# DJjjjhao/FIRA-ICSE

Hardware: NVIDIA B200
Metric: train_commits_per_sec (higher is better)
Workload: dtype bf16

## Files before the change

### fira_icse_b200/csrc/gemm_tc.cu

```cuda
#include <cuda.h>
#include <cudaTypedefs.h>
#include <atomic>
#include <stdlib.h>
#include "common.cuh"
#include "fira_b200.h"

namespace {

constexpr int BM = 128;
constexpr int BK = 64;
constexpr int UMMA_K = 16;
constexpr int NUM_THREADS = 192;

struct TcParams {
  void* C; long ldc; int c_is_bf16;
  int M, N, K;
  const float* bias; const float* rs; const float* rc;
  int relu; int accumulate;
  int splits; int kblocks_per_split;
  int a_kmajor, b_kmajor;
  int rotate;
  int tma_store;
  const __nv_bfloat16* relu_mask;
  float* colsum;
  unsigned long long* probe;
};

std::atomic<unsigned long long*> g_probe{nullptr};

__device__ __forceinline__ void stamp(const TcParams& p, int slot) {
  if (p.probe && blockIdx.x == 0 && blockIdx.y == 0 && blockIdx.z == 0) {
    unsigned long long t;
    asm volatile("mov.u64 %0, %globaltimer;" : "=l"(t));
    p.probe[slot] = t;
  }
}

__device__ __forceinline__ uint32_t smem_addr(const void* p) { return (uint32_t)__cvta_generic_to_shared(p); }

__device__ __forceinline__ void mbar_init(uint32_t bar, uint32_t count) {
  asm volatile("mbarrier.init.shared::cta.b64 [%0], %1;" ::"r"(bar), "r"(count));
}
__device__ __forceinline__ void mbar_expect_tx(uint32_t bar, uint32_t bytes) {
  asm volatile("mbarrier.arrive.expect_tx.shared::cta.b64 _, [%0], %1;" ::"r"(bar), "r"(bytes) : "memory");
}
__device__ __forceinline__ void mbar_wait(uint32_t bar, uint32_t parity) {
  uint32_t ok = 0, spins = 0;
  while (true) {
// ... 9 lines not shown
}
__device__ __forceinline__ void tc_fence_before() { asm volatile("tcgen05.fence::before_thread_sync;" ::: "memory"); }
__device__ __forceinline__ void tc_fence_after() { asm volatile("tcgen05.fence::after_thread_sync;" ::: "memory"); }
__device__ __forceinline__ void umma_commit(uint32_t bar) {
  asm volatile("tcgen05.commit.cta_group::1.mbarrier::arrive::one.shared::cluster.b64 [%0];" ::"r"(bar) : "memory");
}
__device__ __forceinline__ void umma_bf16(uint32_t tmem_d, uint64_t desc_a, uint64_t desc_b, uint32_t idesc,
                                          uint32_t accumulate) {
  asm volatile("{\n\t.reg .pred p;\n\tsetp.ne.b32 p, %4, 0;\n\t"
               "tcgen05.mma.cta_group::1.kind::f16 [%0], %1, %2, %3, p;\n\t}"
               ::"r"(tmem_d), "l"(desc_a), "l"(desc_b), "r"(idesc), "r"(accumulate) : "memory");
}

__device__ __forceinline__ uint64_t make_desc(uint32_t saddr, uint32_t lbo_bytes, uint32_t sbo_bytes) {
  uint64_t d = 0;
  d |= (uint64_t)((saddr >> 4) & 0x3FFF);
  d |= (uint64_t)((lbo_bytes >> 4) & 0x3FFF) << 16;
  d |= (uint64_t)((sbo_bytes >> 4) & 0x3FFF) << 32;
  d |= (uint64_t)1 << 46;
  d |= (uint64_t)2 << 61;
  return d;
}

template <int BN, int STAGES>
__global__ void __launch_bounds__(NUM_THREADS, 2)
gemm_tc_kernel(const __grid_constant__ CUtensorMap tmA, const __grid_constant__ CUtensorMap tmB,
               const __grid_constant__ CUtensorMap tmC, TcParams p) {
  extern __shared__ unsigned char smem_dyn[];
  __shared__ __align__(16) float s_bias[BN], s_rc[BN];
  constexpr uint32_t A_BYTES = BM * BK * 2, B_BYTES = BN * BK * 2, STAGE_BYTES = A_BYTES + B_BYTES;
  __shared__ __align__(8) unsigned long long full_bar[STAGES], empty_bar[STAGES], tmem_full_bar;
  __shared__ uint32_t tmem_base_slot;

  const uint32_t base = (smem_addr(smem_dyn) + 1023u) & ~1023u;
  const int warp = threadIdx.x >> 5, lane = threadIdx.x & 31;
  const int m0 = blockIdx.y * BM, n0 = blockIdx.x * BN;
  const int kb_total = (p.K + BK - 1) / BK;
  const int kb_begin = blockIdx.z * p.kblocks_per_split;
  const int kb_end = min(kb_total, kb_begin + p.kblocks_per_split);
  const int nkb = kb_end - kb_begin;
  if (threadIdx.x == 0) stamp(p, 0);

  const bool do_cs = p.colsum != nullptr && blockIdx.x == 0;
  if (threadIdx.x == 0) {
    for (int s = 0; s < STAGES; ++s) { mbar_init(smem_addr(&full_bar[s]), 1); mbar_init(smem_addr(&empty_bar[s]), do_cs ? 5 : 1); }
    mbar_init(smem_addr(&tmem_full_bar), 1);
    asm volatile("fence.mbarrier_init.release.cluster;" ::: "memory");
    asm volatile("prefetch.tensormap [%0];" ::"l"(&tmA) : "memory");
    asm volatile("prefetch.tensormap [%0];" ::"l"(&tmB) : "memory");
    if (p.tma_store) asm volatile("prefetch.tensormap [%0];" ::"l"(&tmC) : "memory");
  }
  if (warp == 1) {
    asm volatile("tcgen05.alloc.cta_group::1.sync.aligned.shared::cta.b32 [%0], %1;" ::"r"(smem_addr(&tmem_base_slot)), "r"(BN));
    asm volatile("tcgen05.relinquish_alloc_permit.cta_group::1.sync.aligned;");
  }
  tc_fence_before();
  __syncthreads();
  tc_fence_after();
  const uint32_t tmem_acc = tmem_base_slot;
  if (threadIdx.x == 0) stamp(p, 1);
  pdl_wait(); pdl_trigger();
  if (threadIdx.x == 0) stamp(p, 2);

  if (warp == 0 && lane == 0) {
    for (int i = 0; i < nkb; ++i) {
      const int s = i % STAGES;
      const uint32_t ph = (i / STAGES) & 1;
      mbar_wait(smem_addr(&empty_bar[s]), ph ^ 1);
      const uint32_t sa = base + s * STAGE_BYTES, sb = sa + A_BYTES;
      const uint32_t fb = smem_addr(&full_bar[s]);
      mbar_expect_tx(fb, STAGE_BYTES);
      const int kb = p.rotate ? kb_begin + (i + (int)(blockIdx.x + blockIdx.y)) % nkb : kb_begin + i;
      const int k0 = kb * BK;
      if (p.a_kmajor) {
        tma_load_2d(sa, &tmA, k0, m0, fb);
      } else {
        tma_load_2d(sa, &tmA, m0, k0, fb);
        tma_load_2d(sa + 8192, &tmA, m0 + 64, k0, fb);
      }
      if (p.b_kmajor) {
        tma_load_2d(sb, &tmB, k0, n0, fb);
      } else {
#pragma unroll
        for (int j = 0; j < BN / 64; ++j) tma_load_2d(sb + j * 8192, &tmB, n0 + j * 64, k0, fb);
      }
    }
    stamp(p, 3);
  } else if (warp == 1 && lane == 0) {
    const uint32_t idesc = (1u << 4) | (1u << 7) | (1u << 10) | ((p.a_kmajor ? 0u : 1u) << 15) |
                           ((p.b_kmajor ? 0u : 1u) << 16) | ((uint32_t)(BN >> 3) << 17) | ((uint32_t)(BM >> 4) << 24);
    for (int i = 0; i < nkb; ++i) {
      const int s = i % STAGES;
      const uint32_t ph = (i / STAGES) & 1;
      mbar_wait(smem_addr(&full_bar[s]), ph);
      tc_fence_after();
      if (i == 0) stamp(p, 4);
      const uint32_t sa = base + s * STAGE_BYTES, sb = sa + A_BYTES;
#pragma unroll
      for (int k = 0; k < BK / UMMA_K; ++k) {
        const uint64_t da = p.a_kmajor ? make_desc(sa + k * 32, 16, 1024) : make_desc(sa + k * 2048, 8192, 1024);
        const uint64_t db = p.b_kmajor ? make_desc(sb + k * 32, 16, 1024) : make_desc(sb + k * 2048, 8192, 1024);
        umma_bf16(tmem_acc, da, db, idesc, (i > 0 || k > 0) ? 1u : 0u);
      }
      umma_commit(smem_addr(&empty_bar[s]));
    }
    umma_commit(smem_addr(&tmem_full_bar));
    stamp(p, 5);
  } else if (warp >= 2) {
    const int quarter = warp & 3;
    constexpr int HB = BN < 128 ? BN : 128;
    constexpr int PITCH = HB + 4;
    constexpr int LPR = HB / 8;
    constexpr int RPI = 32 / LPR;
    float* stg = reinterpret_cast<float*>(smem_dyn + (base - smem_addr(smem_dyn))) + (size_t)quarter * 32 * PITCH;
    if (do_cs) {
      const int t = quarter * 32 + lane;
      const unsigned char* a_base = smem_dyn + (base - smem_addr(smem_dyn)) + (t >> 6) * 8192 + (t & 7) * 2;
      const int chunk = (t & 63) >> 3;
      float cs = 0.f;
      for (int i = 0; i < nkb; ++i) {
        const int s = i % STAGES;
        mbar_wait(smem_addr(&full_bar[s]), (i / STAGES) & 1);
        const unsigned char* a = a_base + (size_t)s * STAGE_BYTES;
#pragma unroll 8
        for (int k = 0; k < BK; ++k)
          cs += __bfloat162float(*reinterpret_cast<const __nv_bfloat16*>(a + (k >> 3) * 1024 + (k & 7) * 128 + ((chunk ^ (k & 7)) << 4)));
        __syncwarp();
        if (lane == 0) asm volatile("mbarrier.arrive.shared::cta.b64 _, [%0];" ::"r"(smem_addr(&empty_bar[s])) : "memory");
      }
      if (m0 + t < p.M) atomicAdd(p.colsum + m0 + t, cs);
      asm volatile("bar.sync 1, 128;" ::: "memory");
// ... 242 lines not shown
    if (cudaGetDriverEntryPoint("cuTensorMapEncodeTiled", &f, cudaEnableDefault, &q) != cudaSuccess) f = nullptr;
    return (PFN_cuTensorMapEncodeTiled)f;
  }();
  return fn;
}

int make_map(CUtensorMap* map, const void* ptr, long rows, long cols, long ld, int box_cols, int box_rows) {
  PFN_cuTensorMapEncodeTiled enc = get_encode();
  if (!enc) { fira_set_error(FIRA_ERR_CUDA, "gemm_tc: cuTensorMapEncodeTiled unavailable"); return FIRA_ERR_CUDA; }
  cuuint64_t dims[2] = {(cuuint64_t)cols, (cuuint64_t)rows};
  cuuint64_t strides[1] = {(cuuint64_t)ld * 2};
  cuuint32_t box[2] = {(cuuint32_t)box_cols, (cuuint32_t)box_rows};
  cuuint32_t estr[2] = {1, 1};
  CUresult r = enc(map, CU_TENSOR_MAP_DATA_TYPE_BFLOAT16, 2, const_cast<void*>(ptr), dims, strides, box, estr,
                   CU_TENSOR_MAP_INTERLEAVE_NONE, CU_TENSOR_MAP_SWIZZLE_128B, CU_TENSOR_MAP_L2_PROMOTION_L2_128B,
                   CU_TENSOR_MAP_FLOAT_OOB_FILL_NONE);
  if (r != CUDA_SUCCESS) {
    fira_set_error(FIRA_ERR_CUDA, "gemm_tc: cuTensorMapEncodeTiled failed (%d) rows=%ld cols=%ld ld=%ld", (int)r, rows, cols, ld);
    return FIRA_ERR_CUDA;
  }
  return FIRA_OK;
}

template <int BN, int STAGES>
int launch_cfg(const CUtensorMap& ta, const CUtensorMap& tb, const CUtensorMap& tc, const TcParams& p, cudaStream_t st) {
  const size_t smem = (size_t)STAGES * (BM * BK * 2 + BN * BK * 2) + 1024;
  cudaError_t e = cudaFuncSetAttribute(gemm_tc_kernel<BN, STAGES>, cudaFuncAttributeMaxDynamicSharedMemorySize, (int)smem);
  if (e != cudaSuccess) { fira_set_error(FIRA_ERR_CUDA, "gemm_tc attr: %s", cudaGetErrorString(e)); return FIRA_ERR_CUDA; }
  dim3 grid((p.N + BN - 1) / BN, (p.M + BM - 1) / BM, p.splits);
  launch_k(gemm_tc_kernel<BN, STAGES>, dim3(grid), dim3(NUM_THREADS), smem, st, ta, tb, tc, p);
  return FIRA_OK;
}

template <int BN>
int launch(const CUtensorMap& ta, const CUtensorMap& tb, const CUtensorMap& tc, const TcParams& p, cudaStream_t st) {
  const long ctas = (long)((p.N + BN - 1) / BN) * ((p.M + BM - 1) / BM) * p.splits;
  if (ctas > 148) return launch_cfg<BN, (BN == 256 ? 2 : 3)>(ta, tb, tc, p, st);
  return launch_cfg<BN, 4>(ta, tb, tc, p, st);
}

}

extern "C" int fira_debug_set_probe(void* probe) {
  g_probe.store((unsigned long long*)probe, std::memory_order_relaxed);
  return FIRA_OK;
}

namespace {
int gemm_tc_impl(const void* A, long lda, int a_kmajor, const void* B, long ldb, int b_kmajor, void* C, long ldc,
                 int c_is_bf16, int M, int N, int K, const float* bias, const float* rs, const float* rc, int relu,
                 int accumulate, int splits, float* colsum, void* stream, const void* relu_mask = nullptr) {
  FIRA_CHECK_ARG(A && B && C, FIRA_ERR_ARG, "gemm_bf16_tc: null operand");
  FIRA_CHECK_ARG(M > 0 && N > 0 && K > 0, FIRA_ERR_SHAPE, "gemm_bf16_tc: M=%d N=%d K=%d", M, N, K);
  FIRA_CHECK_ARG((lda % 8) == 0 && (ldb % 8) == 0, FIRA_ERR_ALIGN, "gemm_bf16_tc: lda/ldb must be multiples of 8");
  FIRA_CHECK_ARG(fira_aligned16(A) && fira_aligned16(B) && fira_aligned16(C), FIRA_ERR_ALIGN, "gemm_bf16_tc: 16-B alignment");
  FIRA_CHECK_ARG((rs == nullptr) == (rc == nullptr), FIRA_ERR_ARG, "gemm_bf16_tc: rs/rc must come together");
  FIRA_CHECK_ARG(!(splits > 1 && (c_is_bf16 || relu)), FIRA_ERR_ARG, "gemm_bf16_tc: split-K needs fp32 C and no relu");
  cudaStream_t st = (cudaStream_t)stream;
  int BN = N > 128 ? 256 : (N > 64 ? 128 : 64);
  {
    const long mt = (M + BM - 1) / BM;
    const int sp = splits < 1 ? 1 : splits;
    for (int cand = 64; cand < BN; cand *= 2)
      if (mt * ((N + cand - 1) / cand) * sp <= 148) { BN = cand; break; }
  }
  CUtensorMap ta, tb;
  int rc_;
  if (a_kmajor) rc_ = make_map(&ta, A, M, K, lda, BK, BM); else rc_ = make_map(&ta, A, K, M, lda, 64, BK);
  if (rc_) return rc_;
  if (b_kmajor) rc_ = make_map(&tb, B, N, K, ldb, BK, BN); else rc_ = make_map(&tb, B, K, N, ldb, 64, BK);
  if (rc_) return rc_;
  const int kb_total = (K + BK - 1) / BK;
  if (splits < 1) splits = 1;
  if (splits > kb_total) splits = kb_total;
  int per = (kb_total + splits - 1) / splits;
  splits = (kb_total + per - 1) / per;
  const int tma_store = (c_is_bf16 && !accumulate && splits == 1 && (ldc % 8) == 0 && tma_store_on()) ? 1 : 0;
  CUtensorMap tc = ta;
  if (tma_store) {
    rc_ = make_map(&tc, C, M, N, ldc, 64, 32);
    if (rc_) return rc_;
  }
  FIRA_CHECK_ARG(relu_mask == nullptr || tma_store, FIRA_ERR_ARG,
                 "gemm_bf16_tc: the relu mask needs the TMA-store epilogue (bf16 C, no accumulate, no split-K)");
  TcParams p{C, ldc, c_is_bf16, M, N, K, bias, rs, rc, relu, accumulate, splits, per, a_kmajor, b_kmajor, rotate_on() ? 1 : 0,
             tma_store, (const __nv_bfloat16*)relu_mask, colsum,
             g_probe.load(std::memory_order_relaxed)};
  if (splits > 1 && !accumulate) {
    cudaError_t e = cudaMemset2DAsync(C, (size_t)ldc * 4, 0, (size_t)N * 4, (size_t)M, st);
    if (e != cudaSuccess) { fira_set_error(FIRA_ERR_CUDA, "gemm_bf16_tc memset: %s", cudaGetErrorString(e)); return FIRA_ERR_CUDA; }
  }
  if (BN == 256) rc_ = launch<256>(ta, tb, tc, p, st);
  else if (BN == 128) rc_ = launch<128>(ta, tb, tc, p, st);
  else rc_ = launch<64>(ta, tb, tc, p, st);
  if (rc_) return rc_;
  FIRA_CHECK_LAUNCH("fira_gemm_bf16_tc");
  return FIRA_OK;
}
}

extern "C" int fira_gemm_bf16_tc(const void* A, long lda, int a_kmajor, const void* B, long ldb, int b_kmajor, void* C,
                                 long ldc, int c_is_bf16, int M, int N, int K, const float* bias, const float* rs,
                                 const float* rc, int relu, int accumulate, int splits, void* stream) {
  return gemm_tc_impl(A, lda, a_kmajor, B, ldb, b_kmajor, C, ldc, c_is_bf16, M, N, K, bias, rs, rc, relu, accumulate, splits,
                      nullptr, stream);
}

extern "C" int fira_gemm_bf16_tc_dx_relu(const void* dy, long lddy, const void* W, long ldw, void* dx, long lddx,
                                         const void* h, int M, int N, int K, void* stream) {
  FIRA_CHECK_ARG(h != nullptr && fira_aligned16(h), FIRA_ERR_ARG, "gemm_bf16_tc_dx_relu: mask");
  FIRA_CHECK_ARG(tma_store_on(), FIRA_ERR_ARG, "gemm_bf16_tc_dx_relu: needs the TMA-store epilogue (FIRA_GEMM_TMA_STORE=0 is set)");
  return gemm_tc_impl(dy, lddy, 1, W, ldw, 0, dx, lddx, 1, M, N, K, nullptr, nullptr, nullptr, 0, 0, 1, nullptr, stream, h);
}

extern "C" int fira_gemm_bf16_tc_dbias(const void* A, long lda, const void* B, long ldb, int b_kmajor, void* C, long ldc,
                                       int c_is_bf16, int M, int N, int K, int accumulate, int splits, float* d_bias,
                                       void* stream) {
  FIRA_CHECK_ARG(d_bias != nullptr, FIRA_ERR_ARG, "gemm_bf16_tc_dbias: null d_bias");
  return gemm_tc_impl(A, lda, 0, B, ldb, b_kmajor, C, ldc, c_is_bf16, M, N, K, nullptr, nullptr, nullptr, 0, accumulate,
                      splits, d_bias, stream);
}
```

### fira_icse_b200/ops.py

```python
import os

import torch

from . import _lib
from . import optim as _optim
from ._lib import FIRA_BF16, FIRA_F32, call

D = 256

if hasattr(torch.autograd.graph, "set_warn_on_accumulate_grad_stream_mismatch"):
    torch.autograd.graph.set_warn_on_accumulate_grad_stream_mismatch(False)


def _stream():
    return torch.cuda.current_stream().cuda_stream


def _ptr(t, off=0):
    if t is None:
        return None
    return t.data_ptr() + off * t.element_size()


def _require_cuda(*ts):
# ... 154 lines not shown
        if dbias is not None:
            colsum(dy, ld_dy, M, N, x_off=dy_off, out=dbias)
        return gemm_tc(dy, ld_dy, 0, x, ldx, 0, dW, K, N, K, M, splits=splits, a_off=dy_off, b_off=x_off)

    def linear_ln(self, x, W, b, resid, gamma, beta, outA, outB, split, rows, p, seed, sid, rs=None, rc=None):
        N, K = W.shape
        if self.bf16 and N == D and FUSE_GEMM_LN:
            z = torch.empty((rows, D), dtype=torch.bfloat16, device=x.device)
            stats = torch.empty((2, rows), dtype=torch.float32, device=x.device)
            call("fira_gemm_ln_fwd", _ptr(x), K, _ptr(self.w(W)), _ptr(b), _ptr(rs), _ptr(rc), _ptr(resid), _ptr(gamma),
                 _ptr(beta), _ptr(z), _ptr(outA), _ptr(outB) if outB is not outA else None, split, _ptr(stats),
                 _ptr(stats, rows), rows, K, float(p), seed, _ptr(self.seed_ctr), sid, _stream())
            return z, stats
        z = self.linear(x, W, b, rs=rs, rc=rc, M=rows)
        return z, self.ln_fwd(z, resid, gamma, beta, outA, outB, split, rows, p, seed, sid)

    def ln_fwd(self, z, resid, gamma, beta, outA, outB, split, rows, p, seed, sid):
        stats = torch.empty((2, rows), dtype=torch.float32, device=z.device)
        call("fira_ln_residual_fwd", _ptr(z), _ptr(resid), _ptr(gamma), _ptr(beta), _ptr(outA), _ptr(outB), split,
             _ptr(stats), _ptr(stats, rows), rows, D, float(p), seed, _ptr(self.seed_ctr), sid, self.code, _stream())
        return stats

    def ln_bwd(self, dA, dB, split, z, resid, stats, gamma, rows, p, seed, sid, d_resid=None, accum=False, beta=None):
        dz = torch.empty_like(z)
        if d_resid is None:
            d_resid = torch.empty_like(z)
        dgb = _gdest((gamma, beta), (2, D), zero=True) if beta is not None else \
            torch.zeros((2, D), dtype=torch.float32, device=z.device)
        call("fira_ln_residual_bwd", _ptr(dA), _ptr(dB), split, _ptr(z), _ptr(resid), _ptr(stats), _ptr(stats, rows),
             _ptr(gamma), _ptr(dz), _ptr(d_resid), int(accum), _ptr(dgb), _ptr(dgb, D), rows, D, float(p), seed,
             _ptr(self.seed_ctr), sid, self.code, _stream())
        return dz, d_resid, dgb[0], dgb[1]


_F32 = Prec(False)


def ln_fwd(z, resid, gamma, beta, outA, outB, split, rows, p, seed, sid):
    return _F32.ln_fwd(z, resid, gamma, beta, outA, outB, split, rows, p, seed, sid)


def ln_bwd(dA, dB, split, z, resid, stats, gamma, rows, p, seed, sid, d_resid=None, accum=False):
    return _F32.ln_bwd(dA, dB, split, z, resid, stats, gamma, rows, p, seed, sid, d_resid=d_resid, accum=accum)


_SIDE_STREAMS = {}
N_SIDE = max(1, int(os.environ.get("FIRA_SIDE_STREAMS", "8")))
FUSE_GEMM_LN = os.environ.get("FIRA_GEMM_LN", "0") != "0"
FUSE_DX_RELU = os.environ.get("FIRA_DX_RELU", "1") != "0" and os.environ.get("FIRA_GEMM_TMA_STORE", "1") != "0"
MERGE_SPLITS = max(1, int(os.environ.get("FIRA_MERGE_SPLITS", "4")))
_TURN = [0]


class Fork:

    def __init__(self, device, n_side=None):
        self.main = torch.cuda.current_stream(device)
        key = (device.index if device.index is not None else torch.cuda.current_device())
        if key not in _SIDE_STREAMS:
            _SIDE_STREAMS[key] = [torch.cuda.Stream(device=device) for _ in range(N_SIDE)]
        self.sides = _SIDE_STREAMS[key][:n_side] if n_side else _SIDE_STREAMS[key]
        self.side = self.sides[0]
        self.keep = []
        self.used = set()

    def __call__(self, *tensors, lane=None):
        self.keep.extend(tensors)
        if lane is None:
            lane = _TURN[0]
            _TURN[0] += 1
        self.side = self.sides[lane % len(self.sides)]
        self.side.wait_stream(self.main)
# ... 170 lines not shown
        cfg, sou, mark, ast_change, sub_token, edges, rs, B, n_code, n_sub, n_ast, p_comb, p_gcn, fused = ctx.misc
        emb, ast_emb, mark_emb, *lp = ctx.saved_tensors
        N = n_code + n_sub + n_ast
        R, Mc = B * N, B * n_code
        L = len(lp) // ENC_LAYER_PARAMS
        seed, heads = cfg["seed"], cfg["heads"]
        pr = Prec(cfg.get("bf16", False), ctx.wcache, seed_ctr=cfg.get("seed_ctr"))
        dev = emb.device
        f32 = dict(dtype=torch.float32, device=dev)
        st = _stream()
        et = edges.t()
        etrows = et.rows_csr(n_code, n_sub, n_ast) if fused else None
        d_mem = d_mem.contiguous().to(pr.tdt)
        dXc = pr.empty((Mc, D), dev)
        dGin = pr.empty((R, D), dev)
        call("fira_unpack_memory", _ptr(d_mem), _ptr(dXc), _ptr(dGin), B, n_code, n_sub, n_ast, D, pr.code, st)
        d_mark_emb = _gdest(mark_emb, tuple(mark_emb.shape), zero=True)
        grads = [None] * len(lp)
        fork = Fork(dev)
        for i in reversed(range(L)):
            Wq, bq, Wk, bk, Wv, bv, Wo, bo, clw, clb, W1, b1, W2, b2, glw, glb = lp[i * 16:(i + 1) * 16]
            Xc, QK, Vtab, Cd, Zc, st_c, Gin, G, Z, st_g, Wqk, Wc, c1, WcT16 = ctx.saved[i]
            sid = cfg["stream_base"] + i * 8
            dZ, dRes, d_glw, d_glb = pr.ln_bwd(dXc, dGin, Mc, Z, Gin, st_g, glw, R, p_gcn, seed, sid + 2, beta=glb)
            dGin_i = pr.empty((R, D), dev)
            if fused:
                AdZ = pr.empty((R, D), dev)
                call("fira_gcn_layer_bwd", _ptr(etrows[0]), _ptr(etrows[1]), _ptr(etrows[2]), _ptr(dZ), _ptr(WcT16),
                     _ptr(dRes), _ptr(AdZ), _ptr(dGin_i), R, D, st)
            with fork(dZ, G, rs, W1, W2, b1):
                d_b2 = _gdest(b2, (D,), zero=True)
                if fused:
                    fork.keep.append(AdZ)
                    colsum(dZ, D, R, D, out=d_b2)
                    d_c1 = torch.zeros(D, dtype=torch.float32, device=dev)
                    dWc = pr.linear_dw(AdZ, D, Gin, D, R, D, D, dbias=d_c1)
                else:
                    d_c1 = colsum(dZ, D, R, D, weight=rs)
                    dWc = pr.linear_dw(dZ, D, G, D, R, D, D, dbias=d_b2)
                ev_dwc = torch.cuda.Event()
                ev_dwc.record()
                fork.keep.extend((dWc, d_c1))
            with fork():
                torch.cuda.current_stream().wait_event(ev_dwc)
                d_W2 = _gdest(W2, (D, D))
                gemm_raw(_ptr(dWc), D, 1, _ptr(W1), D, 1, _ptr(d_W2), D, D, D, D, rs=d_c1, rc=b1, splits=MERGE_SPLITS if pr.bf16 else 1)
            with fork():
                torch.cuda.current_stream().wait_event(ev_dwc)
                d_W1 = _gdest(W1, (D, D))
                gemm_raw(_ptr(W2), D, 0, _ptr(dWc), D, 0, _ptr(d_W1), D, D, D, D, splits=MERGE_SPLITS if pr.bf16 else 1)
                d_b1 = _gdest(b1, (D,))
                gemm_raw(_ptr(W2), D, 0, _ptr(d_c1), 1, 0, _ptr(d_b1), 1, D, 1, D, splits=1)
            if not fused:
                dG = pr.linear_dx(dZ, D, Wc, R)
                call("fira_gcn_aggregate", _ptr(et.rowptr), _ptr(et.col), _ptr(et.val), _ptr(dG), _ptr(dRes),
                     _ptr(dGin_i), B, n_code, n_sub, n_ast, D, pr.code, st)
            dXc_n = pr.empty((Mc, D), dev)
            dZc, _, d_clw, d_clb = pr.ln_bwd(dGin_i, dGin_i, Mc, Zc, Xc, st_c, clw, Mc, p_comb, seed, sid + 1,
                                             d_resid=dXc_n, beta=clb)
            with fork(dZc, Cd):
                d_bo = _gdest(bo, (D,), zero=True)
                d_Wo = pr.linear_dw(dZc, D, Cd, D, Mc, D, D, out=_gdest(Wo, (D, D)), dbias=d_bo)
            dCd = pr.linear_dx(dZc, D, Wo, Mc)
            dQK = pr.empty((Mc, 2 * D), dev)
            dVtab = torch.zeros((4, D), **f32)
            call("fira_comb_gate_bwd", _ptr(QK), 2 * D, _ptr(Vtab), _ptr(mark), _ptr(dCd), _ptr(dQK), _ptr(dVtab),
                 Mc, D, D // heads, float(p_comb), seed, _ptr(pr.seed_ctr), sid + 0, pr.code, st)
            with fork(dQK, Xc):
                d_bqk = _gdest((bq, bk), (2 * D,), zero=True)
                d_Wqk = pr.linear_dw(dQK, 2 * D, Xc, D, Mc, 2 * D, D, out=_gdest((Wq, Wk), (2 * D, D)), dbias=d_bqk)
            with fork(dVtab, mark_emb, Wv):
                d_Wv = linear_dw(dVtab, D, mark_emb, D, 4, D, D, out=_gdest(Wv, (D, D)))
                d_bv = colsum(dVtab, D, 4, D, out=_gdest(bv, (D,), zero=True))
            with fork(dVtab, Wv, lane=0):
                linear_dx(dVtab, D, Wv, 4, out=d_mark_emb, accumulate=True)
            pr.linear_dx(dQK, 2 * D, Wqk, Mc, out=dXc_n, accumulate=True)
            grads[i * 16:(i + 1) * 16] = [d_Wqk[:D], d_bqk[:D], d_Wqk[D:], d_bqk[D:], d_Wv, d_bv, d_Wo, d_bo,
                                          d_clw, d_clb, d_W1, d_b1, d_W2, d_b2, d_glw, d_glb]
            dXc, dGin = dXc_n, dGin_i
            ctx.saved[i] = None
        d_emb = _gdest(emb, tuple(emb.shape), zero=True)
        d_ast = _gdest(ast_emb, tuple(ast_emb.shape), zero=True)
        call("fira_embed_nodes_bwd", _ptr(sou), _ptr(sub_token), _ptr(ast_change), _ptr(dXc), _ptr(dGin),
             _ptr(d_emb), _ptr(d_ast), B, n_code, n_sub, n_ast, D, pr.code, st)
        fork.join()
        d_mark_emb[0].zero_()
# ... 75 lines not shown
        cfg, tar, memory, mem_mask, tar_mask, KV, Wkv, B, T, S, p, mem_dtype, Ms = ctx.misc
        dec_emb, *lp = ctx.saved_tensors
        Mt = B * T
        pk = cfg.get("packed")
        L = len(lp) // DEC_LAYER_PARAMS
        H, seed = cfg["heads"], cfg["seed"]
        pr = Prec(cfg.get("bf16", False), ctx.wcache, seed_ctr=cfg.get("seed_ctr"))
        dev = dec_emb.device
        st = _stream()
        ldkv = L * 2 * D
        dX = d_out.contiguous().to(pr.tdt).view(Mt, D)
        dKV = pr.empty((Ms, ldkv), dev)
        if pk is not None:
            call("fira_zero_pad_rows", _ptr(dKV), ldkv, ldkv, _ptr(pk.off), B, pk.Rc, pk.Rs, pr.code, st)
        grads = [None] * len(lp)
        F = 4 * D
        fork = Fork(dev)
        for i in reversed(range(L)):
            (sWq, sbq, sWk, sbk, sWv, sbv, sWo, sbo, slw, slb,
             cWq, cbq, cWk, cbk, cWv, cbv, cWo, cbo, clw, clb,
             fW1, fb1, fW2, fb2, flw, flb) = lp[i * 26:(i + 1) * 26]
            X, Wqkv, QKV, ctx1, st1, Z1, ls1, X1, Q, ctx2, st2, Z2, ls2, X2, Hh, Z3, ls3 = ctx.saved[i]
            sid = cfg["stream_base"] + 64 + i * 8
            dZ3, dX2, d_flw, d_flb = pr.ln_bwd(dX, dX, Mt, Z3, X2, ls3, flw, Mt, p, seed, sid + 2, beta=flb)
            with fork(dZ3, Hh):
                d_fb2 = _gdest(fb2, (D,), zero=True)
                d_fW2 = pr.linear_dw(dZ3, D, Hh, F, Mt, D, F, out=_gdest(fW2, (D, F)), dbias=d_fb2)
            dHh = pr.linear_dx_relu(dZ3, D, fW2, Mt, Hh)
            with fork(dHh, X2):
                d_fb1 = _gdest(fb1, (F,), zero=True)
                d_fW1 = pr.linear_dw(dHh, F, X2, D, Mt, F, D, out=_gdest(fW1, (F, D)), dbias=d_fb1)
            pr.linear_dx(dHh, F, fW1, Mt, out=dX2, accumulate=True)
            dZ2, dX1, d_clw, d_clb = pr.ln_bwd(dX2, dX2, Mt, Z2, X1, ls2, clw, Mt, p, seed, sid + 1, beta=clb)
            with fork(dZ2, ctx2):
                d_cbo = _gdest(cbo, (D,), zero=True)
                d_cWo = pr.linear_dw(dZ2, D, ctx2, D, Mt, D, D, out=_gdest(cWo, (D, D)), dbias=d_cbo)
            dctx2 = pr.linear_dx(dZ2, D, cWo, Mt)
            dQ = pr.empty((Mt, D), dev)
            if pk is not None:
                call("fira_attn_packed_bwd", _ptr(Q), D, _ptr(KV, i * 2 * D), ldkv, _ptr(KV, i * 2 * D + D), ldkv,
                     _ptr(pk.ranges), Ms, _ptr(mem_mask), S, pk.chunks, _ptr(ctx2), _ptr(dctx2), D, _ptr(st2), _ptr(dQ), D,
                     _ptr(dKV, i * 2 * D), ldkv, _ptr(dKV, i * 2 * D + D), ldkv, B, H, T, D // H, pr.code, st)
            else:
                call("fira_attn_bwd", _ptr(Q), D, _ptr(KV, i * 2 * D), ldkv, _ptr(KV, i * 2 * D + D), ldkv,
                     _ptr(mem_mask), 0, _ptr(ctx2), _ptr(dctx2), D, _ptr(st2), _ptr(dQ), D, _ptr(dKV, i * 2 * D), ldkv,
                     _ptr(dKV, i * 2 * D + D), ldkv, B, H, T, S, D // H, pr.code, st)
            with fork(dQ, X1):
                d_cbq = _gdest(cbq, (D,), zero=True)
                d_cWq = pr.linear_dw(dQ, D, X1, D, Mt, D, D, out=_gdest(cWq, (D, D)), dbias=d_cbq)
            pr.linear_dx(dQ, D, cWq, Mt, out=dX1, accumulate=True)
            dZ1, dX0, d_slw, d_slb = pr.ln_bwd(dX1, dX1, Mt, Z1, X, ls1, slw, Mt, p, seed, sid + 0, beta=slb)
            with fork(dZ1, ctx1):
                d_sbo = _gdest(sbo, (D,), zero=True)
                d_sWo = pr.linear_dw(dZ1, D, ctx1, D, Mt, D, D, out=_gdest(sWo, (D, D)), dbias=d_sbo)
            dctx1 = pr.linear_dx(dZ1, D, sWo, Mt)
            dQKV = pr.empty((Mt, 3 * D), dev)
            call("fira_attn_bwd", _ptr(QKV), 3 * D, _ptr(QKV, D), 3 * D, _ptr(QKV, 2 * D), 3 * D, _ptr(tar_mask), 1,
                 _ptr(ctx1), _ptr(dctx1), D, _ptr(st1), _ptr(dQKV), 3 * D, _ptr(dQKV, D), 3 * D, _ptr(dQKV, 2 * D), 3 * D,
                 B, H, T, T, D // H, pr.code, st)
            with fork(dQKV, X):
                d_bqkv = _gdest((sbq, sbk, sbv), (3 * D,), zero=True)
                d_Wqkv = pr.linear_dw(dQKV, 3 * D, X, D, Mt, 3 * D, D, out=_gdest((sWq, sWk, sWv), (3 * D, D)), dbias=d_bqkv)
            pr.linear_dx(dQKV, 3 * D, Wqkv, Mt, out=dX0, accumulate=True)
            grads[i * 26:(i + 1) * 26] = [
                d_Wqkv[:D], d_bqkv[:D], d_Wqkv[D:2 * D], d_bqkv[D:2 * D], d_Wqkv[2 * D:], d_bqkv[2 * D:],
                d_sWo, d_sbo, d_slw, d_slb,
                d_cWq, d_cbq, None, None, None, None, d_cWo, d_cbo, d_clw, d_clb,
                d_fW1, d_fb1, d_fW2, d_fb2, d_flw, d_flb]
            dX = dX0
            ctx.saved[i] = None
        mem2 = memory.view(Ms, D)
        with fork(dKV, mem2):
            kv_w = [t for i in range(L) for t in (lp[i * 26 + 12], lp[i * 26 + 14])]
            kv_b = [t for i in range(L) for t in (lp[i * 26 + 13], lp[i * 26 + 15])]
            d_bkv = _gdest(kv_b, (ldkv,), zero=True)
            d_Wkv = pr.linear_dw(dKV, ldkv, mem2, D, Ms, ldkv, D, out=_gdest(kv_w, (ldkv, D)), dbias=d_bkv)
        d_mem = pr.linear_dx(dKV, ldkv, Wkv, Ms).view(memory.shape).to(mem_dtype)
        for i in range(L):
# ... 181 lines not shown
```

### include/fira_b200.h

```cpp
#ifndef FIRA_B200_H_
#define FIRA_B200_H_

#include <stdint.h>

#ifdef __cplusplus
extern "C" {
#endif

#define FIRA_F32 0
#define FIRA_BF16 1
#define FIRA_EDGE_F32 0
#define FIRA_EDGE_BF16 1
#define FIRA_EDGE_F64 2

int fira_version(void);
const char* fira_last_error_string(void);
int fira_built_arch(void);
int fira_set_pdl(int on);
int fira_get_pdl(void);

int fira_gemm_f32(const float* A, long lda, int a_kcontig, const float* B, long ldb, int b_kcontig, float* C,
                  long ldc, int M, int N, int K, const float* bias, const float* rs, const float* rc, int relu,
                  int accumulate, int splits, void* stream);

int fira_gemm_bf16_tc(const void* A, long lda, int a_kmajor, const void* B, long ldb, int b_kmajor, void* C,
                      long ldc, int c_is_bf16, int M, int N, int K, const float* bias, const float* rs,
                      const float* rc, int relu, int accumulate, int splits, void* stream);

int fira_gemm_bf16_tc_dbias(const void* A, long lda, const void* B, long ldb, int b_kmajor, void* C, long ldc,
                            int c_is_bf16, int M, int N, int K, int accumulate, int splits, float* d_bias, void* stream);

int fira_gemm_ln_fwd(const void* x, long ldx, const void* w, const float* bias, const float* rs, const float* rc,
                     const void* resid, const float* gamma, const float* beta, void* z, void* outA, void* outB, long split,
                     float* mean, float* rstd, long rows, int K, float p_drop, uint64_t seed, const uint64_t* seed_ctr,
                     uint32_t stream_id, void* stream);

int fira_gemm_bf16_tc_dx_relu(const void* dy, long lddy, const void* W, long ldw, void* dx, long lddx, const void* h,
                              int M, int N, int K, void* stream);

int fira_debug_set_probe(void* probe);

int fira_embed_nodes_fwd(const int* sou, const int* sub_token, const int* ast_change, const float* emb,
                         const float* ast_emb, const float* pos_table, void* out_code, void* out_rest, int B,
                         int n_code, int n_sub, int n_ast, int dim, int dtype, void* stream);
int fira_embed_nodes_pos_fwd(const int* sou, const int* pos, const int* sub_token, const int* ast_change,
                             const float* emb, const float* ast_emb, const float* pos_table, void* out_code,
                             void* out_rest, int B, int n_code, int n_sub, int n_ast, int dim, int dtype, void* stream);
int fira_zero_pad_rows(void* x, long ld, int width, const int* off, int B, int Rc, int Rs, int dtype, void* stream);
int fira_embed_nodes_bwd(const int* sou, const int* sub_token, const int* ast_change, const void* d_code,
                         const void* d_rest, float* d_emb, float* d_ast_emb, int B, int n_code, int n_sub, int n_ast,
                         int dim, int dtype, void* stream);
int fira_embed_rows_fwd(const int* ids, const float* emb, const float* pos_table, void* out, long rows, int period,
                        int dim, int dtype, void* stream);
int fira_embed_rows_bwd(const int* ids, const void* d_out, float* d_emb, long rows, int dim, int dtype, void* stream);

int fira_ln_residual_fwd(const void* z, const void* resid, const float* gamma, const float* beta, void* outA,
                         void* outB, long split, float* mean, float* rstd, long rows, int dim, float p_drop,
                         uint64_t seed, const uint64_t* seed_ctr, uint32_t stream_id, int dtype, void* stream);
int fira_ln_residual_bwd(const void* d_outA, const void* d_outB, long split, const void* z, const void* resid,
                         const float* mean, const float* rstd, const float* gamma, void* d_z, void* d_resid,
                         int d_resid_accum, float* d_gamma, float* d_beta, long rows, int dim, float p_drop,
// ... 112 lines not shown
```

Baseline: 23850.

## Fuse LayerNorm-residual backward into the following dX tensor-core GEMM prologue

Adds an LN variant of the tcgen05 GEMM kernel. Sixteen producer warps compute the LayerNorm/dropout backward for each 128-row tile and write dz straight into the swizzled A-operand shared-memory stages instead of loading it by TMA. Only the N-block 0 CTA writes dz and d_resid to global memory and accumulates dgamma/dbeta. The Python backward now calls this fused path wherever an ln_bwd is followed by a linear_dx, removing a separate kernel launch and a round trip of dz through global memory. In exchange, the LN backward is recomputed in every N-block CTA, the kernel runs with 512 threads at one CTA per SM, and the path is restricted to K=256 with the TMA-store epilogue and no split-K.

Measured after the change: 20100 (median of 6 runs). -15.7%, worse.

```diff
diff --git a/fira_icse_b200/csrc/gemm_tc.cu b/fira_icse_b200/csrc/gemm_tc.cu
--- a/fira_icse_b200/csrc/gemm_tc.cu
+++ b/fira_icse_b200/csrc/gemm_tc.cu
@@ -3,6 +3,7 @@
 #include <atomic>
 #include <stdlib.h>
 #include "common.cuh"
+#include "tc_common.cuh"
 #include "fira_b200.h"
 
 namespace {
@@ -11,6 +12,18 @@
 constexpr int BK = 64;
 constexpr int UMMA_K = 16;
 constexpr int NUM_THREADS = 192;
+constexpr int LN_PRODUCERS = 16;
+constexpr int LN_THREADS = 32 * LN_PRODUCERS;
+constexpr int LN_D = 256;
+
+struct LnBwd {
+  const __nv_bfloat16* doutA; const __nv_bfloat16* doutB; long split;
+  const __nv_bfloat16* z; const __nv_bfloat16* resid;
+  const float* mean; const float* rstd; const float* gamma;
+  __nv_bfloat16* dz; __nv_bfloat16* dresid; int accum;
+  float* dgamma; float* dbeta;
+  float p_drop; uint64_t seed; const uint64_t* seed_ctr; uint32_t stream_id;
+};
 
 struct TcParams {
   void* C; long ldc; int c_is_bf16;
@@ -24,6 +37,7 @@
   const __nv_bfloat16* relu_mask;
   float* colsum;
   unsigned long long* probe;
+  LnBwd ln;
 };
 
 std::atomic<unsigned long long*> g_probe{nullptr};
@@ -79,8 +93,8 @@
   return d;
 }
 
-template <int BN, int STAGES>
-__global__ void __launch_bounds__(NUM_THREADS, 2)
+template <int BN, int STAGES, bool LN>
+__global__ void __launch_bounds__(LN ? LN_THREADS : NUM_THREADS, LN ? 1 : 2)
 gemm_tc_kernel(const __grid_constant__ CUtensorMap tmA, const __grid_constant__ CUtensorMap tmB,
                const __grid_constant__ CUtensorMap tmC, TcParams p) {
   extern __shared__ unsigned char smem_dyn[];
@@ -88,6 +102,7 @@
   constexpr uint32_t A_BYTES = BM * BK * 2, B_BYTES = BN * BK * 2, STAGE_BYTES = A_BYTES + B_BYTES;
   __shared__ __align__(8) unsigned long long full_bar[STAGES], empty_bar[STAGES], tmem_full_bar;
   __shared__ uint32_t tmem_base_slot;
+  __shared__ __align__(16) float s_dgb[LN ? 2 * LN_D : 4];
 
   const uint32_t base = (smem_addr(smem_dyn) + 1023u) & ~1023u;
   const int warp = threadIdx.x >> 5, lane = threadIdx.x & 31;
@@ -100,7 +115,7 @@
 
   const bool do_cs = p.colsum != nullptr && blockIdx.x == 0;
   if (threadIdx.x == 0) {
-    for (int s = 0; s < STAGES; ++s) { mbar_init(smem_addr(&full_bar[s]), 1); mbar_init(smem_addr(&empty_bar[s]), do_cs ? 5 : 1); }
+    for (int s = 0; s < STAGES; ++s) { mbar_init(smem_addr(&full_bar[s]), LN ? 1 + LN_PRODUCERS : 1); mbar_init(smem_addr(&empty_bar[s]), do_cs ? 5 : 1); }
     mbar_init(smem_addr(&tmem_full_bar), 1);
     asm volatile("fence.mbarrier_init.release.cluster;" ::: "memory");
     asm volatile("prefetch.tensormap [%0];" ::"l"(&tmA) : "memory");
@@ -111,6 +126,7 @@
     asm volatile("tcgen05.alloc.cta_group::1.sync.aligned.shared::cta.b32 [%0], %1;" ::"r"(smem_addr(&tmem_base_slot)), "r"(BN));
     asm volatile("tcgen05.relinquish_alloc_permit.cta_group::1.sync.aligned;");
   }
+  if (LN && threadIdx.x < 2 * LN_D) s_dgb[threadIdx.x] = 0.f;
   tc_fence_before();
   __syncthreads();
   tc_fence_after();
@@ -119,6 +135,117 @@
   pdl_wait(); pdl_trigger();
   if (threadIdx.x == 0) stamp(p, 2);
 
+  auto produce_dz = [&](int pw) {
+    const LnBwd& L = p.ln;
+    uint64_t seed = L.seed;
+    if (L.seed_ctr) seed += *L.seed_ctr;
+    const float keep_scale = L.p_drop > 0.f ? 1.f / (1.f - L.p_drop) : 1.f;
+    const bool writer = blockIdx.x == 0;
+    const int kb = lane >> 3, chunk = lane & 7;
+    const int stage = p.rotate ? (kb - (int)((blockIdx.x + blockIdx.y) % STAGES) + STAGES) % STAGES : kb;
+    unsigned char* a_tile = smem_dyn + (base - smem_addr(smem_dyn)) + (size_t)stage * STAGE_BYTES;
+    float g[8], dg[8], db[8];
+    Act<float>::load8(L.gamma + lane * 8, g);
+#pragma unroll
+    for (int i = 0; i < 8; ++i) { dg[i] = 0.f; db[i] = 0.f; }
+    constexpr int RB = 4;
+    const int row0 = pw * 8;
+#pragma unroll 1
+    for (int r0 = 0; r0 < 8; r0 += RB) {
+      uint4 zr[RB], xr[RB], gr[RB];
+      float mn[RB], rsd[RB];
+#pragma unroll
+      for (int j = 0; j < RB; ++j) {
+        const long m = m0 + row0 + r0 + j;
+        zr[j] = xr[j] = gr[j] = make_uint4(0u, 0u, 0u, 0u);
+        mn[j] = rsd[j] = 0.f;
+        if (m < p.M) {
+          const long o = m * LN_D + lane * 8;
+          zr[j] = *reinterpret_cast<const uint4*>(L.z + o);
+          xr[j] = *reinterpret_cast<const uint4*>(L.resid + o);
+          gr[j] = *reinterpret_cast<const uint4*>((m < L.split ? L.doutA : L.doutB) + o);
+          mn[j] = L.mean[m];
+          rsd[j] = L.rstd[m];
+        }
+      }
+#pragma unroll
+      for (int j = 0; j < RB; ++j) {
+        const long m = m0 + row0 + r0 + j;
+        float y[8], x[8], go[8];
+        const __nv_bfloat162* zh = reinterpret_cast<const __nv_bfloat162*>(&zr[j]);
+        const __nv_bfloat162* xh2 = reinterpret_cast<const __nv_bfloat162*>(&xr[j]);
+        const __nv_bfloat162* gh = reinterpret_cast<const __nv_bfloat162*>(&gr[j]);
+#pragma unroll
+        for (int i = 0; i < 4; ++i) {
+          float2 f = __bfloat1622float2(zh[i]); y[2 * i] = f.x; y[2 * i + 1] = f.y;
+          f = __bfloat1622float2(xh2[i]); x[2 * i] = f.x; x[2 * i + 1] = f.y;
+          f = __bfloat1622float2(gh[i]); go[2 * i] = f.x; go[2 * i + 1] = f.y;
+        }
+        uint32_t mk = 0xffu;
+        if (L.p_drop > 0.f) {
+          mk = dropout_keep8(seed, L.stream_id, (uint64_t)m * 32 + lane, L.p_drop);
+#pragma unroll
+          for (int i = 0; i < 8; ++i) y[i] = ((mk >> i) & 1) ? y[i] * keep_scale : 0.f;
+        }
+        const float mean = mn[j], rstd = rsd[j];
+        float s1 = 0.f, s2 = 0.f;
+#pragma unroll
+        for (int i = 0; i < 8; ++i) {
+          float xh = (y[i] + x[i] - mean) * rstd;
+          float dxh = go[i] * g[i];
+          dg[i] += go[i] * xh; db[i] += go[i];
+          s1 += dxh; s2 += dxh * xh;
+          y[i] = xh; x[i] = dxh;
+        }
+        s1 = warp_sum(s1) * (1.f / LN_D);
+        s2 = warp_sum(s2) * (1.f / LN_D);
+        float dy[8], dz[8];
+#pragma unroll
+        for (int i = 0; i < 8; ++i) {
+          dy[i] = rstd * (x[i] - s1 - y[i] * s2);
+          dz[i] = ((mk >> i) & 1) ? dy[i] * keep_scale : 0.f;
+        }
+        uint4 dzp;
+        __nv_bfloat162* dzh = reinterpret_cast<__nv_bfloat162*>(&dzp);
+#pragma unroll
+        for (int i = 0; i < 4; ++i) dzh[i] = __floats2bfloat162_rn(dz[2 * i], dz[2 * i + 1]);
+        *reinterpret_cast<uint4*>(a_tile + tc::sw128_offset(row0 + r0 + j, chunk)) = dzp;
+        if (writer && m < p.M) {
+          const long o = m * LN_D + lane * 8;
+          *reinterpret_cast<uint4*>(L.dz + o) = dzp;
+          if (L.dresid) {
+            if (L.accum) {
+              float old[8];
+              Act<__nv_bfloat16>::load8(L.dresid + o, old);
+#pragma unroll
+              for (int i = 0; i < 8; ++i) dy[i] += old[i];
+            }
+            Act<__nv_bfloat16>::store8(L.dresid + o, dy);
+          }
+        }
+      }
+    }
+    tc::fence_proxy_async();
+    __syncwarp();
+    if (lane == 0)
+      for (int s = 0; s < STAGES; ++s) tc::mbar_arrive(smem_addr(&full_bar[s]));
+    if (writer) {
+#pragma unroll
+      for (int i = 0; i < 8; ++i) { atomicAdd(&s_dgb[lane * 8 + i], dg[i]); atomicAdd(&s_dgb[LN_D + lane * 8 + i], db[i]); }
+      asm volatile("bar.sync 2, %0;" ::"r"(32 * LN_PRODUCERS) : "memory");
+      const int t = pw * 32 + lane;
+      if (t < 2 * LN_D / 4) {
+        const float4 v = *reinterpret_cast<const float4*>(&s_dgb[t * 4]);
+        float* dst = t < LN_D / 4 ? L.dgamma + t * 4 : L.dbeta + (t * 4 - LN_D);
+        if ((reinterpret_cast<uintptr_t>(dst) & 15u) == 0) {
+          atomicAdd(reinterpret_cast<float4*>(dst), v);
+        } else {
+          atomicAdd(dst, v.x); atomicAdd(dst + 1, v.y); atomicAdd(dst + 2, v.z); atomicAdd(dst + 3, v.w);
+        }
+      }
+    }
+  };
+
   if (warp == 0 && lane == 0) {
     for (int i = 0; i < nkb; ++i) {
       const int s = i % STAGES;
@@ -126,10 +253,11 @@
       mbar_wait(smem_addr(&empty_bar[s]), ph ^ 1);
       const uint32_t sa = base + s * STAGE_BYTES, sb = sa + A_BYTES;
       const uint32_t fb = smem_addr(&full_bar[s]);
-      mbar_expect_tx(fb, STAGE_BYTES);
+      mbar_expect_tx(fb, LN ? B_BYTES : STAGE_BYTES);
       const int kb = p.rotate ? kb_begin + (i + (int)(blockIdx.x + blockIdx.y)) % nkb : kb_begin + i;
       const int k0 = kb * BK;
-      if (p.a_kmajor) {
+      if (LN) {
+      } else if (p.a_kmajor) {
         tma_load_2d(sa, &tmA, k0, m0, fb);
       } else {
         tma_load_2d(sa, &tmA, m0, k0, fb);
@@ -143,6 +271,12 @@
       }
     }
     stamp(p, 3);
+  }
+  if constexpr (LN) {
+    __syncwarp();
+    produce_dz(warp);
+  }
+  if (warp == 0) {
   } else if (warp == 1 && lane == 0) {
     const uint32_t idesc = (1u << 4) | (1u << 7) | (1u << 10) | ((p.a_kmajor ? 0u : 1u) << 15) |
                            ((p.b_kmajor ? 0u : 1u) << 16) | ((uint32_t)(BN >> 3) << 17) | ((uint32_t)(BM >> 4) << 24);
@@ -163,7 +297,7 @@
     }
     umma_commit(smem_addr(&tmem_full_bar));
     stamp(p, 5);
-  } else if (warp >= 2) {
+  } else if (warp >= 2 && warp < 6) {
     const int quarter = warp & 3;
     constexpr int HB = BN < 128 ? BN : 128;
     constexpr int PITCH = HB + 4;
@@ -452,18 +586,19 @@
   return FIRA_OK;
 }
 
-template <int BN, int STAGES>
+template <int BN, int STAGES, bool LN = false>
 int launch_cfg(const CUtensorMap& ta, const CUtensorMap& tb, const CUtensorMap& tc, const TcParams& p, cudaStream_t st) {
   const size_t smem = (size_t)STAGES * (BM * BK * 2 + BN * BK * 2) + 1024;
-  cudaError_t e = cudaFuncSetAttribute(gemm_tc_kernel<BN, STAGES>, cudaFuncAttributeMaxDynamicSharedMemorySize, (int)smem);
+  cudaError_t e = cudaFuncSetAttribute(gemm_tc_kernel<BN, STAGES, LN>, cudaFuncAttributeMaxDynamicSharedMemorySize, (int)smem);
   if (e != cudaSuccess) { fira_set_error(FIRA_ERR_CUDA, "gemm_tc attr: %s", cudaGetErrorString(e)); return FIRA_ERR_CUDA; }
   dim3 grid((p.N + BN - 1) / BN, (p.M + BM - 1) / BM, p.splits);
-  launch_k(gemm_tc_kernel<BN, STAGES>, dim3(grid), dim3(NUM_THREADS), smem, st, ta, tb, tc, p);
+  launch_k(gemm_tc_kernel<BN, STAGES, LN>, dim3(grid), dim3(LN ? LN_THREADS : NUM_THREADS), smem, st, ta, tb, tc, p);
   return FIRA_OK;
 }
 
 template <int BN>
-int launch(const CUtensorMap& ta, const CUtensorMap& tb, const CUtensorMap& tc, const TcParams& p, cudaStream_t st) {
+int launch(const CUtensorMap& ta, const CUtensorMap& tb, const CUtensorMap& tc, const TcParams& p, cudaStream_t st, bool ln) {
+  if (ln) return launch_cfg<BN, 4, true>(ta, tb, tc, p, st);
   const long ctas = (long)((p.N + BN - 1) / BN) * ((p.M + BM - 1) / BM) * p.splits;
   if (ctas > 148) return launch_cfg<BN, (BN == 256 ? 2 : 3)>(ta, tb, tc, p, st);
   return launch_cfg<BN, 4>(ta, tb, tc, p, st);
@@ -479,7 +614,8 @@
 namespace {
 int gemm_tc_impl(const void* A, long lda, int a_kmajor, const void* B, long ldb, int b_kmajor, void* C, long ldc,
                  int c_is_bf16, int M, int N, int K, const float* bias, const float* rs, const float* rc, int relu,
-                 int accumulate, int splits, float* colsum, void* stream, const void* relu_mask = nullptr) {
+                 int accumulate, int splits, float* colsum, void* stream, const void* relu_mask = nullptr,
+                 const LnBwd* ln = nullptr) {
   FIRA_CHECK_ARG(A && B && C, FIRA_ERR_ARG, "gemm_bf16_tc: null operand");
   FIRA_CHECK_ARG(M > 0 && N > 0 && K > 0, FIRA_ERR_SHAPE, "gemm_bf16_tc: M=%d N=%d K=%d", M, N, K);
   FIRA_CHECK_ARG((lda % 8) == 0 && (ldb % 8) == 0, FIRA_ERR_ALIGN, "gemm_bf16_tc: lda/ldb must be multiples of 8");
@@ -515,14 +651,16 @@
                  "gemm_bf16_tc: the relu mask needs the TMA-store epilogue (bf16 C, no accumulate, no split-K)");
   TcParams p{C, ldc, c_is_bf16, M, N, K, bias, rs, rc, relu, accumulate, splits, per, a_kmajor, b_kmajor, rotate_on() ? 1 : 0,
              tma_store, (const __nv_bfloat16*)relu_mask, colsum,
-             g_probe.load(std::memory_order_relaxed)};
+             g_probe.load(std::memory_order_relaxed), ln ? *ln : LnBwd{}};
+  FIRA_CHECK_ARG(ln == nullptr || (tma_store && a_kmajor && !b_kmajor && K == LN_D && splits == 1), FIRA_ERR_ARG,
+                 "gemm_bf16_tc_ln_dx: needs K = 256, the TMA-store epilogue and no split-K");
   if (splits > 1 && !accumulate) {
     cudaError_t e = cudaMemset2DAsync(C, (size_t)ldc * 4, 0, (size_t)N * 4, (size_t)M, st);
     if (e != cudaSuccess) { fira_set_error(FIRA_ERR_CUDA, "gemm_bf16_tc memset: %s", cudaGetErrorString(e)); return FIRA_ERR_CUDA; }
   }
-  if (BN == 256) rc_ = launch<256>(ta, tb, tc, p, st);
-  else if (BN == 128) rc_ = launch<128>(ta, tb, tc, p, st);
-  else rc_ = launch<64>(ta, tb, tc, p, st);
+  if (BN == 256) rc_ = launch<256>(ta, tb, tc, p, st, ln != nullptr);
+  else if (BN == 128) rc_ = launch<128>(ta, tb, tc, p, st, ln != nullptr);
+  else rc_ = launch<64>(ta, tb, tc, p, st, ln != nullptr);
   if (rc_) return rc_;
   FIRA_CHECK_LAUNCH("fira_gemm_bf16_tc");
   return FIRA_OK;
@@ -550,3 +688,24 @@
   return gemm_tc_impl(A, lda, 0, B, ldb, b_kmajor, C, ldc, c_is_bf16, M, N, K, nullptr, nullptr, nullptr, 0, accumulate,
                       splits, d_bias, stream);
 }
+
+extern "C" int fira_gemm_bf16_tc_ln_dx(const void* d_outA, const void* d_outB, long split, const void* z, const void* resid,
+                                       const float* mean, const float* rstd, const float* gamma, void* d_z, void* d_resid,
+                                       int d_resid_accum, float* d_gamma, float* d_beta, float p_drop, uint64_t seed,
+                                       const uint64_t* seed_ctr, uint32_t stream_id, const void* W, long ldw, void* dx,
+                                       long lddx, const void* relu_h, int M, int N, void* stream) {
+  FIRA_CHECK_ARG(d_outA && d_outB && z && resid && mean && rstd && gamma && d_z && d_gamma && d_beta && W && dx, FIRA_ERR_ARG,
+                 "gemm_bf16_tc_ln_dx: null argument");
+  FIRA_CHECK_ARG(fira_aligned16(d_outA) && fira_aligned16(d_outB) && fira_aligned16(z) && fira_aligned16(resid) &&
+                     fira_aligned16(d_z) && fira_aligned16(d_resid) && fira_aligned16(gamma) && fira_aligned16(relu_h),
+                 FIRA_ERR_ALIGN, "gemm_bf16_tc_ln_dx: 16-B alignment");
+  FIRA_CHECK_ARG(p_drop >= 0.f && p_drop < 1.f, FIRA_ERR_ARG, "gemm_bf16_tc_ln_dx: p_drop %f", p_drop);
+  FIRA_CHECK_ARG(d_resid != d_outA && d_resid != d_outB && d_z != d_outA && d_z != d_outB, FIRA_ERR_ARG,
+                 "gemm_bf16_tc_ln_dx: d_z / d_resid must not alias d_out");
+  FIRA_CHECK_ARG(tma_store_on(), FIRA_ERR_ARG, "gemm_bf16_tc_ln_dx: needs the TMA-store epilogue (FIRA_GEMM_TMA_STORE=0 is set)");
+  const LnBwd ln{(const __nv_bfloat16*)d_outA, (const __nv_bfloat16*)d_outB, split, (const __nv_bfloat16*)z,
+                 (const __nv_bfloat16*)resid, mean, rstd, gamma, (__nv_bfloat16*)d_z, (__nv_bfloat16*)d_resid, d_resid_accum,
+                 d_gamma, d_beta, p_drop, seed, seed_ctr, stream_id};
+  return gemm_tc_impl(d_z, LN_D, 1, W, ldw, 0, dx, lddx, 1, M, N, LN_D, nullptr, nullptr, nullptr, 0, 0, 1, nullptr, stream,
+                      relu_h, &ln);
+}
diff --git a/fira_icse_b200/ops.py b/fira_icse_b200/ops.py
--- a/fira_icse_b200/ops.py
+++ b/fira_icse_b200/ops.py
@@ -200,15 +200,35 @@
         return stats
 
     def ln_bwd(self, dA, dB, split, z, resid, stats, gamma, rows, p, seed, sid, d_resid=None, accum=False, beta=None):
+        dz, d_resid, dgb = self._ln_bwd_out(z, gamma, beta, d_resid)
+        call("fira_ln_residual_bwd", _ptr(dA), _ptr(dB), split, _ptr(z), _ptr(resid), _ptr(stats), _ptr(stats, rows),
+             _ptr(gamma), _ptr(dz), _ptr(d_resid), int(accum), _ptr(dgb), _ptr(dgb, D), rows, D, float(p), seed,
+             _ptr(self.seed_ctr), sid, self.code, _stream())
+        return dz, d_resid, dgb[0], dgb[1]
+
+    @staticmethod
+    def _ln_bwd_out(z, gamma, beta, d_resid):
         dz = torch.empty_like(z)
         if d_resid is None:
             d_resid = torch.empty_like(z)
         dgb = _gdest((gamma, beta), (2, D), zero=True) if beta is not None else \
             torch.zeros((2, D), dtype=torch.float32, device=z.device)
-        call("fira_ln_residual_bwd", _ptr(dA), _ptr(dB), split, _ptr(z), _ptr(resid), _ptr(stats), _ptr(stats, rows),
-             _ptr(gamma), _ptr(dz), _ptr(d_resid), int(accum), _ptr(dgb), _ptr(dgb, D), rows, D, float(p), seed,
-             _ptr(self.seed_ctr), sid, self.code, _stream())
-        return dz, d_resid, dgb[0], dgb[1]
+        return dz, d_resid, dgb
+
+    def ln_bwd_dx(self, dA, dB, split, z, resid, stats, gamma, rows, p, seed, sid, W, relu_h=None, d_resid=None,
+                  accum=False, beta=None):
+        if not (self.bf16 and FUSE_LN_DX and (relu_h is None or FUSE_DX_RELU)):
+            dz, d_resid, dg, db = self.ln_bwd(dA, dB, split, z, resid, stats, gamma, rows, p, seed, sid, d_resid=d_resid,
+                                              accum=accum, beta=beta)
+            dx = self.linear_dx(dz, D, W, rows) if relu_h is None else self.linear_dx_relu(dz, D, W, rows, relu_h)
+            return dz, d_resid, dg, db, dx
+        N = W.shape[1]
+        dz, d_resid, dgb = self._ln_bwd_out(z, gamma, beta, d_resid)
+        dx = torch.empty((rows, N), dtype=torch.bfloat16, device=z.device)
+        call("fira_gemm_bf16_tc_ln_dx", _ptr(dA), _ptr(dB), split, _ptr(z), _ptr(resid), _ptr(stats), _ptr(stats, rows),
+             _ptr(gamma), _ptr(dz), _ptr(d_resid), int(accum), _ptr(dgb), _ptr(dgb, D), float(p), seed, _ptr(self.seed_ctr),
+             sid, _ptr(self.w(W)), N, _ptr(dx), N, _ptr(relu_h), rows, N, _stream())
+        return dz, d_resid, dgb[0], dgb[1], dx
 
 
 _F32 = Prec(False)
@@ -226,6 +246,7 @@
 N_SIDE = max(1, int(os.environ.get("FIRA_SIDE_STREAMS", "8")))
 FUSE_GEMM_LN = os.environ.get("FIRA_GEMM_LN", "0") != "0"
 FUSE_DX_RELU = os.environ.get("FIRA_DX_RELU", "1") != "0" and os.environ.get("FIRA_GEMM_TMA_STORE", "1") != "0"
+FUSE_LN_DX = os.environ.get("FIRA_LN_DX", "1") != "0" and os.environ.get("FIRA_GEMM_TMA_STORE", "1") != "0"
 MERGE_SPLITS = max(1, int(os.environ.get("FIRA_MERGE_SPLITS", "4")))
 _TURN = [0]
 
@@ -442,7 +463,11 @@
             Wq, bq, Wk, bk, Wv, bv, Wo, bo, clw, clb, W1, b1, W2, b2, glw, glb = lp[i * 16:(i + 1) * 16]
             Xc, QK, Vtab, Cd, Zc, st_c, Gin, G, Z, st_g, Wqk, Wc, c1, WcT16 = ctx.saved[i]
             sid = cfg["stream_base"] + i * 8
-            dZ, dRes, d_glw, d_glb = pr.ln_bwd(dXc, dGin, Mc, Z, Gin, st_g, glw, R, p_gcn, seed, sid + 2, beta=glb)
+            if fused:
+                dZ, dRes, d_glw, d_glb = pr.ln_bwd(dXc, dGin, Mc, Z, Gin, st_g, glw, R, p_gcn, seed, sid + 2, beta=glb)
+            else:
+                dZ, dRes, d_glw, d_glb, dG = pr.ln_bwd_dx(dXc, dGin, Mc, Z, Gin, st_g, glw, R, p_gcn, seed, sid + 2, Wc,
+                                                          beta=glb)
             dGin_i = pr.empty((R, D), dev)
             if fused:
                 AdZ = pr.empty((R, D), dev)
@@ -472,16 +497,14 @@
                 d_b1 = _gdest(b1, (D,))
                 gemm_raw(_ptr(W2), D, 0, _ptr(d_c1), 1, 0, _ptr(d_b1), 1, D, 1, D, splits=1)
             if not fused:
-                dG = pr.linear_dx(dZ, D, Wc, R)
                 call("fira_gcn_aggregate", _ptr(et.rowptr), _ptr(et.col), _ptr(et.val), _ptr(dG), _ptr(dRes),
                      _ptr(dGin_i), B, n_code, n_sub, n_ast, D, pr.code, st)
             dXc_n = pr.empty((Mc, D), dev)
-            dZc, _, d_clw, d_clb = pr.ln_bwd(dGin_i, dGin_i, Mc, Zc, Xc, st_c, clw, Mc, p_comb, seed, sid + 1,
-                                             d_resid=dXc_n, beta=clb)
+            dZc, _, d_clw, d_clb, dCd = pr.ln_bwd_dx(dGin_i, dGin_i, Mc, Zc, Xc, st_c, clw, Mc, p_comb, seed, sid + 1, Wo,
+                                                     d_resid=dXc_n, beta=clb)
             with fork(dZc, Cd):
                 d_bo = _gdest(bo, (D,), zero=True)
                 d_Wo = pr.linear_dw(dZc, D, Cd, D, Mc, D, D, out=_gdest(Wo, (D, D)), dbias=d_bo)
-            dCd = pr.linear_dx(dZc, D, Wo, Mc)
             dQK = pr.empty((Mc, 2 * D), dev)
             dVtab = torch.zeros((4, D), **f32)
             call("fira_comb_gate_bwd", _ptr(QK), 2 * D, _ptr(Vtab), _ptr(mark), _ptr(dCd), _ptr(dQK), _ptr(dVtab),
@@ -603,20 +626,19 @@
              fW1, fb1, fW2, fb2, flw, flb) = lp[i * 26:(i + 1) * 26]
             X, Wqkv, QKV, ctx1, st1, Z1, ls1, X1, Q, ctx2, st2, Z2, ls2, X2, Hh, Z3, ls3 = ctx.saved[i]
             sid = cfg["stream_base"] + 64 + i * 8
-            dZ3, dX2, d_flw, d_flb = pr.ln_bwd(dX, dX, Mt, Z3, X2, ls3, flw, Mt, p, seed, sid + 2, beta=flb)
+            dZ3, dX2, d_flw, d_flb, dHh = pr.ln_bwd_dx(dX, dX, Mt, Z3, X2, ls3, flw, Mt, p, seed, sid + 2, fW2, relu_h=Hh,
+                                                       beta=flb)
             with fork(dZ3, Hh):
                 d_fb2 = _gdest(fb2, (D,), zero=True)
                 d_fW2 = pr.linear_dw(dZ3, D, Hh, F, Mt, D, F, out=_gdest(fW2, (D, F)), dbias=d_fb2)
-            dHh = pr.linear_dx_relu(dZ3, D, fW2, Mt, Hh)
             with fork(dHh, X2):
                 d_fb1 = _gdest(fb1, (F,), zero=True)
                 d_fW1 = pr.linear_dw(dHh, F, X2, D, Mt, F, D, out=_gdest(fW1, (F, D)), dbias=d_fb1)
             pr.linear_dx(dHh, F, fW1, Mt, out=dX2, accumulate=True)
-            dZ2, dX1, d_clw, d_clb = pr.ln_bwd(dX2, dX2, Mt, Z2, X1, ls2, clw, Mt, p, seed, sid + 1, beta=clb)
+            dZ2, dX1, d_clw, d_clb, dctx2 = pr.ln_bwd_dx(dX2, dX2, Mt, Z2, X1, ls2, clw, Mt, p, seed, sid + 1, cWo, beta=clb)
             with fork(dZ2, ctx2):
                 d_cbo = _gdest(cbo, (D,), zero=True)
                 d_cWo = pr.linear_dw(dZ2, D, ctx2, D, Mt, D, D, out=_gdest(cWo, (D, D)), dbias=d_cbo)
-            dctx2 = pr.linear_dx(dZ2, D, cWo, Mt)
             dQ = pr.empty((Mt, D), dev)
             if pk is not None:
                 call("fira_attn_packed_bwd", _ptr(Q), D, _ptr(KV, i * 2 * D), ldkv, _ptr(KV, i * 2 * D + D), ldkv,
@@ -630,11 +652,10 @@
                 d_cbq = _gdest(cbq, (D,), zero=True)
                 d_cWq = pr.linear_dw(dQ, D, X1, D, Mt, D, D, out=_gdest(cWq, (D, D)), dbias=d_cbq)
             pr.linear_dx(dQ, D, cWq, Mt, out=dX1, accumulate=True)
-            dZ1, dX0, d_slw, d_slb = pr.ln_bwd(dX1, dX1, Mt, Z1, X, ls1, slw, Mt, p, seed, sid + 0, beta=slb)
+            dZ1, dX0, d_slw, d_slb, dctx1 = pr.ln_bwd_dx(dX1, dX1, Mt, Z1, X, ls1, slw, Mt, p, seed, sid + 0, sWo, beta=slb)
             with fork(dZ1, ctx1):
                 d_sbo = _gdest(sbo, (D,), zero=True)
                 d_sWo = pr.linear_dw(dZ1, D, ctx1, D, Mt, D, D, out=_gdest(sWo, (D, D)), dbias=d_sbo)
-            dctx1 = pr.linear_dx(dZ1, D, sWo, Mt)
             dQKV = pr.empty((Mt, 3 * D), dev)
             call("fira_attn_bwd", _ptr(QKV), 3 * D, _ptr(QKV, D), 3 * D, _ptr(QKV, 2 * D), 3 * D, _ptr(tar_mask), 1,
                  _ptr(ctx1), _ptr(dctx1), D, _ptr(st1), _ptr(dQKV), 3 * D, _ptr(dQKV, D), 3 * D, _ptr(dQKV, 2 * D), 3 * D,
diff --git a/include/fira_b200.h b/include/fira_b200.h
--- a/include/fira_b200.h
+++ b/include/fira_b200.h
@@ -37,6 +37,12 @@
 
 int fira_gemm_bf16_tc_dx_relu(const void* dy, long lddy, const void* W, long ldw, void* dx, long lddx, const void* h,
                               int M, int N, int K, void* stream);
+
+int fira_gemm_bf16_tc_ln_dx(const void* d_outA, const void* d_outB, long split, const void* z, const void* resid,
+                            const float* mean, const float* rstd, const float* gamma, void* d_z, void* d_resid,
+                            int d_resid_accum, float* d_gamma, float* d_beta, float p_drop, uint64_t seed,
+                            const uint64_t* seed_ctr, uint32_t stream_id, const void* W, long ldw, void* dx, long lddx,
+                            const void* relu_h, int M, int N, void* stream);
 
 int fira_debug_set_probe(void* probe);
 
```
